# csteinmetz1/dasp-pytorch

Hardware: NVIDIA H100
Metric: audio samples/sec (fwd+bwd) @ batch=1024x2chx48k (higher is better)
Workload: dtype f32

## Files before the change

### dasp_pytorch_b200/csrc/reverb.cu

```cuda
#include <cufft.h>
#include <curand_kernel.h>
#include <math.h>

#include <map>
#include <mutex>
#include <tuple>
#include <vector>

#include "common.cuh"
#include "fft8192.cuh"

namespace dasp {
namespace {

constexpr int kBands = 12;
constexpr int kB = 4096;
constexpr int kNbA = 2 * kB;
constexpr double kPi = 3.14159265358979323846;

#define DASP_CUFFT_OK(expr)                                                        \
  do {                                                                             \
    cufftResult r__ = (expr);                                                      \
    if (r__ != CUFFT_SUCCESS) {                                                    \
      ::dasp::set_error("%s failed: cufft error %d (%s:%d)", #expr, (int)r__, __FILE__, __LINE__); \
// ... 784 lines not shown
  FftSmem s(sm);
  __shared__ float red[kFusedThreads / 32][2 * kBands];
  __shared__ float rk[kBands];
  __shared__ int cls_lo[17], cls_off[17];
  const int t = threadIdx.x;
  s.init(twiddles, t);
  const fft8k::Tables tb = fft8k::carve_tables(s.tabf);
  auto fetch = [&](int it, int m) {
    if (t != 0 || m >= nunits) return;
    uint64_t* bar = &s.full[it & 1];
    float* dst = s.G + (it & 1) * 2 * fft8k::kPlaneG;
    const float* src = Epl + (int64_t)m * 2 * kNbA;
    mbar_arrive_expect_tx(bar, 2u * kNbA * 4u);
#pragma unroll
    for (int q = 0; q < 4; ++q) tma_load_1d(dst + q * 4096, src + q * 4096, 16384u, bar);
  };
  fetch(0, blockIdx.x);
  fetch(1, blockIdx.x + gridDim.x);
  const float step = 1.0f / (float)(L - 1);
  float2* D = reinterpret_cast<float2*>(s.Yr);
  int it = 0;
  for (int m = blockIdx.x; m < nunits; m += gridDim.x, ++it) {
    mbar_wait(&s.full[it & 1], (uint32_t)((it >> 1) & 1));
    float* gr = s.G + (it & 1) * 2 * fft8k::kPlaneG;
    const int64_t il = m / J;
    const int j = m - (int)il * J;
    const int lo = j * kB, hi = (lo + kB < leff) ? lo + kB : leff;
    float xr[16], xi[16];
    fft8192_in_smem<true>(gr, gr + fft8k::kPlaneG, s, tb, t, [&] { fetch(it + 2, m + 2 * gridDim.x); }, [] {}, xr, xi);
    __syncthreads();
    if (t < kBands) rk[t] = -(params[il * 25 + kBands + t] * 10.0f + 1.0f);
    if (t == 0) {
      int off = 0;
      for (int c = 0; c < R; ++c) {
        const int a_lo = (lo - c + R - 1) / R, a_hi = (hi - c + R - 1) / R;
        cls_lo[c] = a_lo;
        cls_off[c] = off;
        off += (a_hi > a_lo) ? a_hi - a_lo : 0;
      }
      cls_off[R] = off;
    }
#pragma unroll
    for (int q = 0; q < 8; ++q) D[t + 512 * q] = make_float2(xr[q], xi[q]);
    __syncthreads();
    float s0[kBands], s1[kBands];
#pragma unroll
    for (int k = 0; k < kBands; ++k) { s0[k] = 0.f; s1[k] = 0.f; }
    const float2* cb = C + (il * kBands) * (int64_t)R * nb;
    const int ntaps = cls_off[R];
    for (int idx = t; idx < ntaps; idx += kFusedThreads) {
      int c = 0;
      while (c + 1 < R && idx >= cls_off[c + 1]) ++c;
      const int a = cls_lo[c] + (idx - cls_off[c]);
      const int tau = R * a + c;
      const float2 gd = D[tau - lo];
      const float tt = time_axis32(tau, L, step);
      const float2* c0 = cb + (int64_t)c * nb + a;
      float2 v[kBands];
#pragma unroll
      for (int k = 0; k < kBands; ++k) v[k] = c0[(int64_t)k * R * nb];
#pragma unroll
      for (int k = 0; k < kBands; ++k) {
        const float w = fmaf(gd.x, v[k].x, gd.y * v[k].y) * __expf(rk[k] * tt);
        s0[k] += w;
        s1[k] = fmaf(w, tt, s1[k]);
      }
    }
    const int lane = t & 31, warp = t >> 5;
#pragma unroll
    for (int k = 0; k < kBands; ++k) {
      const float x0 = warp_sum(s0[k]), x1 = warp_sum(s1[k]);
      if (lane == 0) { red[warp][2 * k] = x0; red[warp][2 * k + 1] = x1; }
    }
    __syncthreads();
    if (t < 2 * kBands) {
      float acc = 0.f;
#pragma unroll
      for (int w = 0; w < kFusedThreads / 32; ++w) acc += red[w][t];
      part[((int64_t)m * kBands) * 2 + t] = acc;
    }
  }
}

constexpr int kMaxFusedR = 8;

__device__ __forceinline__ unsigned cluster_ctarank() {
  unsigned r;
  asm volatile("mov.u32 %0, %%cluster_ctarank;" : "=r"(r));
  return r;
}
__device__ __forceinline__ void cluster_arrive() { asm volatile("barrier.cluster.arrive.release;" ::: "memory"); }
__device__ __forceinline__ void cluster_wait() { asm volatile("barrier.cluster.wait.acquire;" ::: "memory"); }
__device__ __forceinline__ float* map_to_cta(float* smem_ptr, unsigned rank) {
  uint64_t r;
  asm volatile("mapa.u64 %0, %1, %2;" : "=l"(r) : "l"(reinterpret_cast<uint64_t>(smem_ptr)), "r"(rank));
  return reinterpret_cast<float*>(r);
}

template <int R>
__global__ void __launch_bounds__(kFusedThreads, 1)
ir_synth_fused_kernel(const float2* __restrict__ H1, const float* __restrict__ twiddles,
                      const float* __restrict__ params, float2* __restrict__ Hb, float2* __restrict__ Csave, int64_t item0, int64_t L, int64_t leff, int jb,
                      const unsigned long long* seed) {
  constexpr int nb = fft8k::kN, U = nb / 2 + 1, CT = R * kFusedThreads, total = kBands * U;
  static_assert(CT < U, "at most one band may complete per generation round");
  extern __shared__ __align__(16) float sm[];
  float* G = sm;
  float* Yr = sm + 4 * fft8k::kPlaneG;
  float* Yi = Yr + fft8k::kPlaneY;
  float* tabf = Yi + fft8k::kPlaneY;
  float* gk = tabf + fft8k::kTabFloats;
  float* rk = gk + 16;
  const int t = threadIdx.x;
  const unsigned c = cluster_ctarank();
  const int64_t il = blockIdx.y;

  for (int e = t; e < fft8k::kTabFloats; e += kFusedThreads) tabf[e] = twiddles[e];
  if (t < kBands) {
    gk[t] = params[il * 25 + t] * (1.0f / kBands);
    rk[t] = -(params[il * 25 + kBands + t] * 10.0f + 1.0f);
  }
  const fft8k::Tables tb = fft8k::carve_tables(tabf);
  float* remote[R];
#pragma unroll
  for (int b = 0; b < R; ++b) remote[b] = map_to_cta(G, (unsigned)b);
  const PhiloxKeys keys = philox_keys(__ldg(seed));
  const float step = 1.0f / (float)(L - 1);
  float accr[16], acci[16];
#pragma unroll
  for (int q = 0; q < 16; ++q) { accr[q] = 0.f; acci[q] = 0.f; }
  cluster_arrive();
  cluster_wait();

  int processed = 0;
  bool buffer_handed_back = false;
  constexpr int rounds = (total + CT - 1) / CT;
  for (int r = 0; r < rounds; ++r) {
    if (buffer_handed_back) { cluster_wait(); buffer_handed_back = false; }
    const int u = r * CT + (int)c * kFusedThreads + t;
    if (u < total) {
      const int k = u / U, j1 = u - k * U;
      const unsigned long long pair = (unsigned long long)((item0 + il) * kBands + k);
      const bool self_mirror = (j1 == 0) || (2 * j1 == nb);
      const int off = (k & 1) * 2 * fft8k::kPlaneG;
      spectral_unit<R>(j1, nb, H1 + (int64_t)k * (R * nb / 2 + 1), pair, keys, [&](int b, float2 q, float2 qm) {
        float* base = remote[b] + off;
        base[j1] = q.x;
        base[fft8k::kPlaneG + j1] = q.y;
        if (!self_mirror) {
          base[nb - j1] = qm.x;
          base[fft8k::kPlaneG + nb - j1] = qm.y;
        }
      });
    }
    const int done = (r + 1) * CT < total ? (r + 1) * CT : total;
    if (done / U > processed) {
      cluster_arrive();
      cluster_wait();
      const int kk = processed;
      float* gr = G + (kk & 1) * 2 * fft8k::kPlaneG;
      float* gi = gr + fft8k::kPlaneG;
      fft8k::p1<true>(gr, gi, tb, t);
      __syncthreads();
      fft8k::p2<true>(gr, gi, Yr, Yi, tb, t);
      __syncthreads();
      cluster_arrive();
      buffer_handed_back = true;
      fft8k::P3Regs q3;
      fft8k::p3_load<true>(Yr, Yi, t, q3);
      __syncthreads();
      fft8k::p3_store<true>(Yr, Yi, tb, t, q3);
      __syncthreads();
      float xr[16], xi[16];
      fft8k::p4<true>(Yr, Yi, t, xr, xi);
      const float g = gk[kk], rr = rk[kk];
      float2* fout = Csave ? Csave + ((il * kBands + kk) * R + c) * (int64_t)nb : nullptr;
#pragma unroll
      for (int q = 0; q < 16; ++q) {
        const int a = t + 512 * q;
        const float e = g * __expf(rr * time_axis((int64_t)R * a + c, L, step));
        accr[q] = fmaf(e, xr[q], accr[q]);
        acci[q] = fmaf(e, xi[q], acci[q]);
        if (fout) fout[a] = make_float2(xr[q], xi[q]);
      }
      ++processed;
    }
  }
  if (buffer_handed_back) cluster_wait();
  float2* out = Hb + il * (int64_t)jb * kNbA;
#pragma unroll
  for (int q = 0; q < 16; ++q) {
    const int64_t tau = (int64_t)R * (t + 512 * q) + c;
    if (tau < leff) out[(tau / kB) * kNbA + (tau % kB)] = make_float2(accr[q], acci[q]);
  }
}

__global__ void ir_grad_pp_kernel(const float2* __restrict__ Et, const float2* __restrict__ C,
                                  const float* __restrict__ params, float* __restrict__ part, int64_t L, int64_t leff,
                                  int jb, int R, int nb) {
  const int64_t il = blockIdx.y;
  __shared__ float rk[kBands];
  __shared__ float red[8][2 * kBands];
  if (threadIdx.x < kBands) rk[threadIdx.x] = -(params[il * 25 + kBands + threadIdx.x] * 10.0f + 1.0f);
  __syncthreads();
  const float step = 1.0f / (float)(L - 1);
  const float2* de = Et + il * (int64_t)jb * kNbA;
  const float2* cb = C + (il * kBands) * (int64_t)R * nb;
  float s0[kBands], s1[kBands];
#pragma unroll
  for (int k = 0; k < kBands; ++k) { s0[k] = 0.f; s1[k] = 0.f; }
  const int stride = gridDim.x * blockDim.x;
  for (int t = blockIdx.x * blockDim.x + threadIdx.x; t < leff; t += 2 * stride) {
    const int t2 = t + stride;
    const bool has2 = t2 < leff;
    const int a = t / R, ph = t - a * R;
    const int a2 = has2 ? t2 / R : a, ph2 = has2 ? t2 - a2 * R : ph;
    const float2 gd = de[(t / kB) * kNbA + (t % kB)];
    const float2 gd2 = has2 ? de[(t2 / kB) * kNbA + (t2 % kB)] : make_float2(0.f, 0.f);
    const float2* c0 = cb + (int64_t)ph * nb + a;
    const float2* c1 = cb + (int64_t)ph2 * nb + a2;
    float2 v[kBands], v2[kBands];
#pragma unroll
    for (int k = 0; k < kBands; ++k) { v[k] = c0[(int64_t)k * R * nb]; v2[k] = c1[(int64_t)k * R * nb]; }
    const float tt = time_axis(t, L, step), tt2 = time_axis(has2 ? t2 : t, L, step);
#pragma unroll
    for (int k = 0; k < kBands; ++k) {
      const float w = fmaf(gd.x, v[k].x, gd.y * v[k].y) * __expf(rk[k] * tt);
      const float w2 = fmaf(gd2.x, v2[k].x, gd2.y * v2[k].y) * __expf(rk[k] * tt2);
      s0[k] += w + w2;
      s1[k] = fmaf(w, tt, fmaf(w2, tt2, s1[k]));
    }
  }
  const int lane = threadIdx.x & 31, warp = threadIdx.x >> 5;
#pragma unroll
  for (int k = 0; k < kBands; ++k) {
    const float x0 = warp_sum(s0[k]), x1 = warp_sum(s1[k]);
    if (lane == 0) { red[warp][2 * k] = x0; red[warp][2 * k + 1] = x1; }
  }
  __syncthreads();
  if (threadIdx.x < 2 * kBands) {
    float acc = 0.f;
    for (int w = 0; w < (int)(blockDim.x >> 5); ++w) acc += red[w][threadIdx.x];
    part[((il * gridDim.x + blockIdx.x) * kBands) * 2 + threadIdx.x] = acc;
  }
}


__global__ void x_blocks_kernel(const float* __restrict__ x, float2* __restrict__ Xb, int64_t item0, int I, int64_t n,
                                int in_chs) {
  const int i = blockIdx.x;
  const int64_t il = blockIdx.y;
  const float* xl = x + ((item0 + il) * in_chs) * n;
  const float* xr = in_chs == 1 ? xl : xl + n;
  float2* out = Xb + (il * I + i) * (int64_t)kNbA;
  for (int m = threadIdx.x; m < kNbA; m += blockDim.x) {
    const int64_t idx = (int64_t)(i - 1) * kB + m;
    float2 v = make_float2(0.f, 0.f);
    if (idx >= 0 && idx < n) v = make_float2(xl[idx], xr[idx]);
    out[m] = v;
  }
}

__device__ __forceinline__ void untangle(float2 z, float2 zm, float2& a, float2& b) {
  a = make_float2(0.5f * (z.x + zm.x), 0.5f * (z.y - zm.y));
  b = make_float2(0.5f * (z.y + zm.y), -0.5f * (z.x - zm.x));
}
__device__ __forceinline__ void cfma(float2& acc, float2 p, float2 q) {
  acc.x = fmaf(p.x, q.x, fmaf(-p.y, q.y, acc.x));
  acc.y = fmaf(p.x, q.y, fmaf(p.y, q.x, acc.y));
}
__device__ __forceinline__ void cfma_conj(float2& acc, float2 p, float2 q) {
  acc.x = fmaf(p.x, q.x, fmaf(p.y, q.y, acc.x));
  acc.y = fmaf(p.y, q.x, fmaf(-p.x, q.y, acc.y));
}

template <int MAXB, bool CORR, bool PLANAR = false>
__global__ void __launch_bounds__(128) partition_mac_kernel(const float2* __restrict__ A, const float2* __restrict__ Bm,
// ... 372 lines not shown
  for (int k = 0; k < kBands; ++k)
    for (int64_t i = 0; i < g.taps; ++i) padded[(size_t)k * n1 + i] = taps[(size_t)k * g.taps + i] * inv;
  float* d_in = nullptr;
  cufftComplex* d_out = nullptr;
  void* d_work = nullptr;
  DASP_CUDA_OK(cudaMalloc(&d_in, sizeof(float) * padded.size()));
  DASP_CUDA_OK(cudaMalloc(&d_out, sizeof(cufftComplex) * kBands * n1c));
  DASP_CUDA_OK(cudaMemcpyAsync(d_in, padded.data(), sizeof(float) * padded.size(), cudaMemcpyHostToDevice, st));
  PlanVal pv;
  int rc = get_plan(0, n1, kBands, n1, n1c, pv);
  if (rc != DASP_OK) return rc;
  DASP_CUDA_OK(cudaMalloc(&d_work, pv.work > 0 ? pv.work : 16));
  DASP_CUFFT_OK(cufftSetStream(pv.h, st));
  DASP_CUFFT_OK(cufftSetWorkArea(pv.h, d_work));
  DASP_CUFFT_OK(cufftExecR2C(pv.h, d_in, d_out));
  DASP_CUDA_OK(cudaStreamSynchronize(st));
  cudaFree(d_in);
  cudaFree(d_work);
  g_fb[key] = d_out;
  *out = reinterpret_cast<const float2*>(d_out);
  return DASP_OK;
}

template <int R>
void launch_spectral(float2* C, const float2* H1, int64_t item0, int64_t items, int nb, const unsigned long long* seed,
                     bool planar, cudaStream_t st) {
  const int threads = 128;
  dim3 grid((unsigned)((nb / 2 + 1 + threads - 1) / threads), kBands, (unsigned)items);
  if (planar) spectral_gen_kernel<R, true><<<grid, threads, 0, st>>>(C, H1, item0, nb, seed);
  else        spectral_gen_kernel<R, false><<<grid, threads, 0, st>>>(C, H1, item0, nb, seed);
}
bool dispatch_spectral(int R, float2* C, const float2* H1, int64_t item0, int64_t items, int nb,
                       const unsigned long long* seed, bool planar, cudaStream_t st) {
  switch (R) {
#define DASP_R(r) case r: launch_spectral<r>(C, H1, item0, items, nb, seed, planar, st); return true;
    DASP_R(1) DASP_R(2) DASP_R(3) DASP_R(4) DASP_R(5) DASP_R(6) DASP_R(7) DASP_R(8) DASP_R(9) DASP_R(10)
    DASP_R(11) DASP_R(12) DASP_R(13) DASP_R(14) DASP_R(15) DASP_R(16)
#undef DASP_R
    default: return false;
  }
}
constexpr int kMaxSpectralR = 16;

std::map<int, float*> g_fft_tab;
int get_fft_tables(cudaStream_t st, const float** out) {
  int dev = 0;
  DASP_CUDA_OK(cudaGetDevice(&dev));
  auto it = g_fft_tab.find(dev);
  if (it == g_fft_tab.end()) {
    std::vector<float> h(fft8k::kTabFloats, 0.f);
    for (int e = 0; e < fft8k::kTabEntries; ++e) {
      int co, so, dup;
      double turns;
      fft8k::table_entry(e, co, so, dup, turns);
      const float c = (float)cos(2.0 * kPi * turns), sn = (float)sin(2.0 * kPi * turns);
      h[co] = c; h[so] = sn;
      if (dup) { h[co + 1] = c; h[so + 1] = sn; }
    }
    float* d = nullptr;
    DASP_CUDA_OK(cudaMalloc(&d, sizeof(float) * h.size()));
    DASP_CUDA_OK(cudaMemcpyAsync(d, h.data(), sizeof(float) * h.size(), cudaMemcpyHostToDevice, st));
    DASP_CUDA_OK(cudaStreamSynchronize(st));
    it = g_fft_tab.emplace(dev, d).first;
  }
  *out = it->second;
  return DASP_OK;
}
int configure_fft_kernels();
int launch_ifft_shape(float2* C, const float* tw, const float* params, float2* hs, bool save_f, int64_t items,
                      const Geom& g, int jb, cudaStream_t st) {
  int rc = configure_fft_kernels();
  if (rc != DASP_OK) return rc;
  const size_t smem = kFftSmemBytes;
  ifft_shape_kernel<<<dim3((unsigned)g.rpp, (unsigned)items), kFusedThreads, smem, st>>>(
      reinterpret_cast<float*>(C), tw, params, hs, save_f ? 1 : 0, (int)g.L, (int)g.leff, jb, (int)g.rpp);
  DASP_LAUNCH_OK("ifft_shape_kernel");
  return DASP_OK;
}
int g_last_fused = 0;
std::map<std::pair<int, int>, int> g_fused_ok;
template <int R>
bool launch_fused(const float2* H1, const float* tw, const float* params, float2* hs, float2* Csave, int64_t item0, int64_t items,
                  int64_t L, int64_t leff, int jb, const unsigned long long* seed, cudaStream_t st) {
  auto kern = ir_synth_fused_kernel<R>;
  const size_t smem = sizeof(float) * kFusedSmemFloats;
  cudaLaunchConfig_t cfg = {};
  cfg.gridDim = dim3(R, (unsigned)items, 1);
  cfg.blockDim = dim3(kFusedThreads, 1, 1);
  cfg.dynamicSmemBytes = smem;
  cfg.stream = st;
  cudaLaunchAttribute at[1];
  at[0].id = cudaLaunchAttributeClusterDimension;
  at[0].val.clusterDim.x = R; at[0].val.clusterDim.y = 1; at[0].val.clusterDim.z = 1;
  cfg.attrs = at;
  cfg.numAttrs = 1;
  int dev = 0;
  cudaGetDevice(&dev);
  auto it = g_fused_ok.find({dev, R});
  if (it == g_fused_ok.end()) {
    int n = 0;
    if (cudaFuncSetAttribute(kern, cudaFuncAttributeMaxDynamicSharedMemorySize, (int)smem) != cudaSuccess ||
        cudaOccupancyMaxActiveClusters(&n, kern, &cfg) != cudaSuccess) {
      n = 0;
      cudaGetLastError();
    }
    it = g_fused_ok.emplace(std::make_pair(dev, R), n).first;
  }
  if (it->second < 1) return false;
  cudaLaunchKernelEx(&cfg, kern, H1, tw, params, hs, Csave, item0, L, leff, jb, seed);
  return true;
}
bool dispatch_fused(int R, const float2* H1, const float* tw, const float* params, float2* hs, float2* Csave, int64_t item0,
                    int64_t items, int64_t L, int64_t leff, int jb, const unsigned long long* seed, cudaStream_t st) {
  switch (R) {
#define DASP_R(r) case r: return launch_fused<r>(H1, tw, params, hs, Csave, item0, items, L, leff, jb, seed, st);
    DASP_R(1) DASP_R(2) DASP_R(3) DASP_R(4) DASP_R(5) DASP_R(6) DASP_R(7) DASP_R(8)
#undef DASP_R
    default: return false;
  }
}

inline size_t align256(size_t v) { return (v + 255) & ~(size_t)255; }

struct FwdWs { size_t ys, xsp, hsp, extra, cufft, total; };
struct BwdWs { size_t gs, ds, es, extra, mixpart, cufft, total; };

void fwd_layout(const ConvGeom& g, size_t extra_bytes, size_t cufft_work, FwdWs& w) {
  size_t o = 0;
  w.ys = o;  o += align256(sizeof(float2) * (size_t)(g.chunk * g.ib * kNbA));
  w.xsp = o; o += align256(sizeof(float2) * (size_t)(g.chunk * g.ib * kNbA));
  w.hsp = o; o += align256(sizeof(float2) * (size_t)(g.chunk * g.jb * kNbA));
  w.extra = o; o += align256(extra_bytes);
  w.cufft = o; o += align256(cufft_work);
  w.total = o;
}
void bwd_layout(const ConvGeom& g, size_t extra_bytes, size_t cufft_work, BwdWs& w) {
  size_t o = 0;
  w.gs = o; o += align256(sizeof(float2) * (size_t)(g.chunk * g.ib * kNbA));
  w.ds = o; o += align256(sizeof(float2) * (size_t)(g.chunk * g.ib * kNbA));
  w.es = o; o += align256(sizeof(float2) * (size_t)(g.chunk * g.jb * kNbA));
  w.extra = o; o += align256(extra_bytes);
  w.mixpart = o; o += align256(sizeof(float) * (size_t)(g.chunk * g.ib));
  w.cufft = o; o += align256(cufft_work);
  w.total = o;
}

struct Plans { PlanVal xi, hj, blk, pp; };
struct Setup { Plans full, rem; FwdWs fwd; BwdWs bwd; };
int conv_setup(const ConvGeom& g, const Geom* synth, Setup& s) {
  int rc;
  size_t work = 0;
  for (int64_t items : {g.bs > 0 ? g.chunk : 0, g.bs % g.chunk}) {
    if (items == 0) continue;
    Plans& p = items == g.chunk ? s.full : s.rem;
    if ((rc = get_plan(2, kNbA, items * g.ib, kNbA, kNbA, p.xi)) != DASP_OK) return rc;
    if ((rc = get_plan(2, kNbA, items * g.jb, kNbA, kNbA, p.hj)) != DASP_OK) return rc;
    if (p.xi.work > work) work = p.xi.work;
    if (p.hj.work > work) work = p.hj.work;
    if (synth) {
      if ((rc = get_plan(2, synth->nb, items * kBands * synth->nbk, synth->nb, synth->nb, p.blk)) != DASP_OK) return rc;
      if ((rc = get_plan(2, synth->nb, items * kBands * synth->rpp, synth->nb, synth->nb, p.pp)) != DASP_OK) return rc;
      if (p.blk.work > work) work = p.blk.work;
      if (p.pp.work > work) work = p.pp.work;
    }
  }
  size_t fwd_extra = 0, bwd_extra = 0;
  if (synth) {
    fwd_extra = sizeof(float2) * (size_t)(g.chunk * kBands * synth->pair_c64());
    int64_t nparts = synth->nbk > synth->nparts_pp() ? synth->nbk : synth->nparts_pp();
    if (g.jb > nparts) nparts = g.jb;
    bwd_extra = sizeof(float) * (size_t)(g.chunk * nparts * kBands * 2);
  }
  fwd_layout(g, fwd_extra, work, s.fwd);
  bwd_layout(g, bwd_extra, work, s.bwd);
  return DASP_OK;
}
int check_workspace(const char* what, size_t need, int64_t have) {
  if ((int64_t)need > have) {
    set_error("%s: workspace needs %lld bytes, got %lld", what, (long long)need, (long long)have);
    return DASP_ERR_WORKSPACE;
  }
  return DASP_OK;
}

template <class Out>
int put_conv_geometry(const ConvGeom& g, const Geom* synth, Out* out) {
  std::lock_guard<std::mutex> lk(g_mu);
  Setup s{};
  int rc = conv_setup(g, synth, s);
  if (rc != DASP_OK) return rc;
  out->leff = g.leff; out->conv_block = kB; out->x_blocks = g.ib; out->ir_partitions = g.jb; out->chunk_items = g.chunk;
  out->xspec_c64 = g.bs * g.ib * kNbA;
  out->irspec_c64 = g.bs * g.jb * kNbA;
  out->fwd_workspace_bytes = (int64_t)s.fwd.total;
  out->bwd_workspace_bytes = (int64_t)s.bwd.total;
  return DASP_OK;
}

template <bool CORR, bool PLANAR = false>
// ... 132 lines not shown
}

}

void reverb_shutdown() {
  std::lock_guard<std::mutex> lk(g_mu);
  for (auto& kv : g_plans) cufftDestroy(kv.second.h);
  g_plans.clear();
  for (auto& kv : g_fb) cudaFree(kv.second);
  g_fb.clear();
  for (auto& kv : g_fft_tab) cudaFree(kv.second);
  g_fft_tab.clear();
}

}

using namespace dasp;

extern "C" {

int dasp_debug_reverb_last_path(void) { return g_last_fused; }

int dasp_reverb_filterbank(int64_t taps, double sample_rate, float* out) {
  DASP_REQUIRE(out != nullptr && taps >= 1 && (taps % 2) == 1, "filterbank: taps must be odd and out non-null");
  DASP_REQUIRE(sample_rate / 2.0 > 18000.0, "filterbank: needs 18 kHz < sample_rate/2");
  std::vector<float> v;
  octave_filterbank((int)taps, sample_rate, v);
  for (size_t i = 0; i < v.size(); ++i) out[i] = v[i];
  return DASP_OK;
}

int dasp_reverb_geometry(int64_t bs, int64_t n, int64_t num_samples, int64_t taps, int64_t chunk_items,
                         dasp_reverb_geom* out) {
  DASP_REQUIRE(out != nullptr, "reverb geometry: null out");
  Geom g;
  int rc = make_geom(bs, n, num_samples, taps, chunk_items, g);
  if (rc != DASP_OK) return rc;
  if ((rc = put_conv_geometry(g, &g, out)) != DASP_OK) return rc;
  out->nb = g.nb; out->hop = g.hop; out->nbk = g.nbk; out->rpp = g.rpp;
  out->f_floats = bs * kBands * g.pair_c64() * 2;
  return DASP_OK;
}

int dasp_reverb_fwd(const float* x, int64_t in_chs, const float* params, const float* noise, const uint64_t* seed_dev, float* y,
                    float* f_save, void* xspec_save, void* irspec_save, void* workspace,
                    int64_t workspace_bytes, int64_t bs, int64_t n, int64_t num_samples, int64_t taps,
                    int64_t chunk_items, float sample_rate, void* stream) {
  Geom g;
  int rc = make_geom(bs, n, num_samples, taps, chunk_items, g);
  if (rc != DASP_OK) return rc;
  DASP_REQUIRE(in_chs == 1 || in_chs == 2, "only mono/stereo signals are supported");
  if (bs == 0) return DASP_OK;
  DASP_REQUIRE(x && params && y && workspace, "reverb fwd: null pointer");
  DASP_REQUIRE(noise != nullptr || seed_dev != nullptr, "reverb fwd: device-noise mode needs seed_dev (a device pointer)");
  const unsigned long long* seed = reinterpret_cast<const unsigned long long*>(seed_dev);
  cudaStream_t st = (cudaStream_t)stream;
  std::lock_guard<std::mutex> lk(g_mu);
  const float2 *H = nullptr, *H1 = nullptr;
  const bool spectral = (noise == nullptr) && g.rpp <= kMaxSpectralR;
  if (spectral) { if ((rc = get_filterbank_n1(g, (double)sample_rate, st, &H1)) != DASP_OK) return rc; }
  else          { if ((rc = get_filterbank(g, (double)sample_rate, st, &H)) != DASP_OK) return rc; }
  Setup s{};
  if ((rc = conv_setup(g, &g, s)) != DASP_OK) return rc;
  if ((rc = check_workspace("reverb fwd", s.fwd.total, workspace_bytes)) != DASP_OK) return rc;
  const FwdWs& w = s.fwd;
  unsigned char* base = (unsigned char*)workspace;
  void* ws_cufft = base + w.cufft;
  const int64_t lp = g.L + g.P;
  const int nbk = (int)g.nbk, nb = (int)g.nb, hop = (int)g.hop, P = (int)g.P, I = (int)g.ib, J = (int)g.jb;

  for (int64_t item0 = 0; item0 < bs; item0 += g.chunk) {
    const int64_t items = (bs - item0 < g.chunk) ? bs - item0 : g.chunk;
    const Plans& pl = (items == g.chunk) ? s.full : s.rem;
    float2* C = f_save ? reinterpret_cast<float2*>(f_save) + item0 * kBands * g.pair_c64()
                       : reinterpret_cast<float2*>(base + w.extra);
    float2* xs = xspec_save ? (float2*)xspec_save + item0 * I * (int64_t)kNbA : (float2*)(base + w.xsp);
    float2* hs = irspec_save ? (float2*)irspec_save + item0 * J * (int64_t)kNbA : (float2*)(base + w.hsp);
    const dim3 gblk((unsigned)nbk, kBands, (unsigned)items);
    const bool own_conv = own_fft_rows(n, x, hs);

    if (!own_conv) DASP_CUDA_OK(cudaMemsetAsync(hs, 0, sizeof(float2) * items * J * kNbA, st));
    int synth = 0;
    const bool own_fft = spectral && nb == fft8k::kN && g.L < (int64_t)1 << 31;
    if (own_fft && debug_reverb_path() == 2 && g.rpp <= kMaxFusedR) synth = 1;
    else if (own_fft && debug_reverb_path() != 1) synth = 2;
    const float* tw = nullptr;
    if ((synth != 0 || own_conv) && (rc = get_fft_tables(st, &tw)) != DASP_OK) return rc;
    if (synth == 1) {
      if (dispatch_fused((int)g.rpp, H1, tw, params + item0 * 25, hs, f_save ? C : nullptr, item0, items, g.L, g.leff, J,
                         seed, st)) {
        DASP_LAUNCH_OK("ir_synth_fused_kernel");
      } else {
        synth = 2;
      }
    }
    g_last_fused = synth;
    if (synth == 1) {
    } else if (synth == 2) {
      dispatch_spectral((int)g.rpp, C, H1, item0, items, nb, seed, true, st);
      DASP_LAUNCH_OK("spectral_gen_kernel");
      if ((rc = launch_ifft_shape(C, tw, params + item0 * 25, hs, f_save != nullptr, items, g, J, st)) != DASP_OK) return rc;
    } else if (spectral) {
      dispatch_spectral((int)g.rpp, C, H1, item0, items, nb, seed, false, st);
      DASP_LAUNCH_OK("spectral_gen_kernel");
      DASP_CUFFT_OK(cufftSetStream(pl.pp.h, st));
      DASP_CUFFT_OK(cufftSetWorkArea(pl.pp.h, ws_cufft));
      DASP_CUFFT_OK(cufftExecC2C(pl.pp.h, (cufftComplex*)C, (cufftComplex*)C, CUFFT_INVERSE));
      shape_ir_pp_kernel<<<dim3((unsigned)((g.leff + 255) / 256), (unsigned)items), 256, 0, st>>>(
          C, params + item0 * 25, hs, g.L, g.leff, J, (int)g.rpp, nb);
      DASP_LAUNCH_OK("shape_ir_pp_kernel");
    } else {
      if (noise) noise_pairs_layout_kernel<<<gblk, 256, 0, st>>>(noise, C, item0, nbk, nb, hop, lp);
      else       noise_pairs_philox_kernel<<<gblk, 256, 0, st>>>(C, item0, nbk, nb, hop, seed);
      DASP_LAUNCH_OK("reverb noise kernel");
      DASP_CUFFT_OK(cufftSetStream(pl.blk.h, st));
      DASP_CUFFT_OK(cufftSetWorkArea(pl.blk.h, ws_cufft));
      DASP_CUFFT_OK(cufftExecC2C(pl.blk.h, (cufftComplex*)C, (cufftComplex*)C, CUFFT_FORWARD));
      cmul_filter_pairs_kernel<<<gblk, 256, 0, st>>>(C, H, nbk, nb);
      DASP_LAUNCH_OK("cmul_filter_pairs_kernel");
      DASP_CUFFT_OK(cufftExecC2C(pl.blk.h, (cufftComplex*)C, (cufftComplex*)C, CUFFT_INVERSE));
      shape_ir_pairs_kernel<<<dim3((unsigned)nbk, (unsigned)items), 256, 0, st>>>(C, params + item0 * 25, hs, g.L, g.leff,
                                                                               J, nbk, nb, hop, P);
      DASP_LAUNCH_OK("shape_ir_pairs_kernel");
    }
    if ((rc = conv_fwd_chunk(g, pl, own_conv, tw, x, (int)in_chs, xs, hs, params + 24, 25, y, base, w, item0, items,
                             st)) != DASP_OK)
      return rc;
  }
  return DASP_OK;
}

int dasp_reverb_bwd(const float* gy, const float* x, int64_t in_chs, const float* params,
                    const float* f_save, const void* xspec_save, const void* irspec_save, float* gx, float* gparams,
                    void* workspace, int64_t workspace_bytes, int64_t bs, int64_t n, int64_t num_samples, int64_t taps,
                    int64_t chunk_items, int64_t device_noise, void* stream) {
  Geom g;
  int rc = make_geom(bs, n, num_samples, taps, chunk_items, g);
  if (rc != DASP_OK) return rc;
  DASP_REQUIRE(in_chs == 1 || in_chs == 2, "only mono/stereo signals are supported");
  if (bs == 0) return DASP_OK;
  const bool polyphase = device_noise != 0 && g.rpp <= kMaxSpectralR;
  DASP_REQUIRE(gy && x && params && f_save && xspec_save && irspec_save && gx && gparams && workspace,
               "reverb bwd: null pointer");
  cudaStream_t st = (cudaStream_t)stream;
  std::lock_guard<std::mutex> lk(g_mu);
  Setup s{};
  if ((rc = conv_setup(g, &g, s)) != DASP_OK) return rc;
  if ((rc = check_workspace("reverb bwd", s.bwd.total, workspace_bytes)) != DASP_OK) return rc;
  const BwdWs& w = s.bwd;
  unsigned char* base = (unsigned char*)workspace;
  const float2* ws_es = (const float2*)(base + w.es);
  float* ws_irpart = (float*)(base + w.extra);
  const float* ws_mixpart = (const float*)(base + w.mixpart);
  const int nbk = (int)g.nbk, nb = (int)g.nb, hop = (int)g.hop, P = (int)g.P, I = (int)g.ib, J = (int)g.jb;

  for (int64_t item0 = 0; item0 < bs; item0 += g.chunk) {
    const int64_t items = (bs - item0 < g.chunk) ? bs - item0 : g.chunk;
    const Plans& pl = (items == g.chunk) ? s.full : s.rem;
    const float2* C = reinterpret_cast<const float2*>(f_save) + item0 * kBands * g.pair_c64();
    const float2* xs = (const float2*)xspec_save + item0 * I * (int64_t)kNbA;
    const float2* hs = (const float2*)irspec_save + item0 * J * (int64_t)kNbA;

    const bool own_conv = own_fft_rows(n, gy, nullptr);
    const bool own_irgrad = own_conv && polyphase && nb == fft8k::kN && g.L < (int64_t)1 << 31;
    const float* tw = nullptr;
    if (own_conv && (rc = get_fft_tables(st, &tw)) != DASP_OK) return rc;
    if ((rc = conv_bwd_chunk(g, pl, own_conv, own_irgrad ? IrGrad::kPlanar : IrGrad::kTime, tw, gy, x, (int)in_chs, xs,
                             hs, params + 24, 25, gx, base, w, item0, items, st)) != DASP_OK)
      return rc;
    int nparts;
    if (own_irgrad) {
      nparts = J;
      const int nunits = (int)(items * J);
      const unsigned ig_grid = (unsigned)(nunits < sm_count() ? nunits : sm_count());
      ifft_irgrad_kernel<<<ig_grid, kFusedThreads, kFftSmemBytes, st>>>(reinterpret_cast<const float*>(ws_es), tw, C,
                                                                        params + item0 * 25, ws_irpart, (int)g.L,
                                                                        (int)g.leff, J, (int)g.rpp, nunits);
      DASP_LAUNCH_OK("ifft_irgrad_kernel");
    } else {
      if (polyphase) {
        nparts = (int)g.nparts_pp();
// ... 123 lines not shown
```

Measured before the change: 4.560 billion.

## Warp-specialize cluster IR synthesis with async remote stores and mbarrier double-buffering

Replaces the fused IR synthesis kernel with a warp-specialized cluster kernel. Dedicated generator warps, with reduced registers via setmaxnreg, write spectral bins into peer CTAs' shared memory using st.async with mbarrier transaction counts. FFT warps consume double-buffered bands signalled by full/empty mbarriers instead of cluster-wide barriers, and the kernel is persistent across items with the grid capped by max active clusters. It also replaces per-element expf with a recurrence for the decay envelope. It becomes the default path for rpp<=6 instead of the two-kernel spectral+iFFT path, which adds complexity and occupancy risk.

```diff
diff --git a/dasp_pytorch_b200/csrc/reverb.cu b/dasp_pytorch_b200/csrc/reverb.cu
--- a/dasp_pytorch_b200/csrc/reverb.cu
+++ b/dasp_pytorch_b200/csrc/reverb.cu
@@ -890,117 +890,173 @@
   }
 }
 
-constexpr int kMaxFusedR = 8;
-
+constexpr int kMaxClusterR = 6;
+constexpr int kSynthGen = 384, kSynthThreads = kFusedThreads + kSynthGen;
+constexpr int kSynthFftRegs = 80, kSynthGenRegs = 56;
+constexpr int kMaxHookR = 8;
+constexpr size_t kSynthSmemBytes =
+    sizeof(float) * (2 * 2 * fft8k::kPlaneG + 2 * fft8k::kPlaneY + fft8k::kTabFloats) + 4 * sizeof(uint64_t);
+
+__device__ __forceinline__ void cluster_arrive() { asm volatile("barrier.cluster.arrive.release;" ::: "memory"); }
+__device__ __forceinline__ void cluster_wait() { asm volatile("barrier.cluster.wait.acquire;" ::: "memory"); }
 __device__ __forceinline__ unsigned cluster_ctarank() {
   unsigned r;
   asm volatile("mov.u32 %0, %%cluster_ctarank;" : "=r"(r));
   return r;
 }
-__device__ __forceinline__ void cluster_arrive() { asm volatile("barrier.cluster.arrive.release;" ::: "memory"); }
-__device__ __forceinline__ void cluster_wait() { asm volatile("barrier.cluster.wait.acquire;" ::: "memory"); }
-__device__ __forceinline__ float* map_to_cta(float* smem_ptr, unsigned rank) {
-  uint64_t r;
-  asm volatile("mapa.u64 %0, %1, %2;" : "=l"(r) : "l"(reinterpret_cast<uint64_t>(smem_ptr)), "r"(rank));
-  return reinterpret_cast<float*>(r);
-}
+__device__ __forceinline__ uint32_t mapa_u32(uint32_t smem_addr, uint32_t rank) {
+  uint32_t r;
+  asm("mapa.shared::cluster.u32 %0, %1, %2;" : "=r"(r) : "r"(smem_addr), "r"(rank));
+  return r;
+}
+__device__ __forceinline__ void st_async(uint32_t addr, float v, uint32_t bar) {
+  asm volatile("st.async.shared::cluster.mbarrier::complete_tx::bytes.b32 [%0], %1, [%2];" ::"r"(addr),
+               "r"(__float_as_uint(v)), "r"(bar)
+               : "memory");
+}
+__device__ __forceinline__ void mbar_arrive_remote(uint32_t cluster_bar) {
+  asm volatile("mbarrier.arrive.relaxed.cluster.shared::cluster.b64 _, [%0];" ::"r"(cluster_bar) : "memory");
+}
+__device__ __forceinline__ void fence_cluster() { asm volatile("fence.acq_rel.cluster;" ::: "memory"); }
+__device__ __forceinline__ void mbar_wait_cluster(uint64_t* bar, uint32_t parity) {
+  uint32_t done;
+  do {
+    asm volatile(
+        "{\n.reg .pred p;\n"
+        "mbarrier.try_wait.parity.acquire.cluster.shared::cta.b64 p, [%1], %2;\n"
+        "selp.u32 %0, 1, 0, p;\n}\n"
+        : "=r"(done)
+        : "r"(smem_u32(bar)), "r"(parity)
+        : "memory");
+  } while (!done);
+}
+__device__ __forceinline__ void fft_sync() { asm volatile("bar.sync 1, %0;" ::"n"(kFusedThreads) : "memory"); }
 
 template <int R>
-__global__ void __launch_bounds__(kFusedThreads, 1)
-ir_synth_fused_kernel(const float2* __restrict__ H1, const float* __restrict__ twiddles,
-                      const float* __restrict__ params, float2* __restrict__ Hb, float2* __restrict__ Csave, int64_t item0, int64_t L, int64_t leff, int jb,
-                      const unsigned long long* seed) {
-  constexpr int nb = fft8k::kN, U = nb / 2 + 1, CT = R * kFusedThreads, total = kBands * U;
-  static_assert(CT < U, "at most one band may complete per generation round");
-  extern __shared__ __align__(16) float sm[];
+__global__ void __launch_bounds__(kSynthThreads, 1)
+ir_synth_cluster_kernel(const float2* __restrict__ H1, const float* __restrict__ twiddles, const float* __restrict__ params,
+                        float2* __restrict__ Hb, float2* __restrict__ Csave, int64_t item0, int items, int L, int leff,
+                        int jb, const unsigned long long* seed) {
+  constexpr int nb = fft8k::kN, U = nb / 2 + 1, NG = kSynthGen, NT = kSynthThreads;
+  constexpr int CT = R * NG, total = kBands * U;
+  constexpr uint32_t kBandBytes = 2u * nb * 4u;
+  extern __shared__ __align__(128) float sm[];
   float* G = sm;
   float* Yr = sm + 4 * fft8k::kPlaneG;
   float* Yi = Yr + fft8k::kPlaneY;
   float* tabf = Yi + fft8k::kPlaneY;
-  float* gk = tabf + fft8k::kTabFloats;
-  float* rk = gk + 16;
+  uint64_t* full = reinterpret_cast<uint64_t*>(tabf + fft8k::kTabFloats);
+  uint64_t* empty = full + 2;
   const int t = threadIdx.x;
   const unsigned c = cluster_ctarank();
-  const int64_t il = blockIdx.y;
-
-  for (int e = t; e < fft8k::kTabFloats; e += kFusedThreads) tabf[e] = twiddles[e];
-  if (t < kBands) {
-    gk[t] = params[il * 25 + t] * (1.0f / kBands);
-    rk[t] = -(params[il * 25 + kBands + t] * 10.0f + 1.0f);
-  }
-  const fft8k::Tables tb = fft8k::carve_tables(tabf);
-  float* remote[R];
-#pragma unroll
-  for (int b = 0; b < R; ++b) remote[b] = map_to_cta(G, (unsigned)b);
-  const PhiloxKeys keys = philox_keys(__ldg(seed));
-  const float step = 1.0f / (float)(L - 1);
-  float accr[16], acci[16];
-#pragma unroll
-  for (int q = 0; q < 16; ++q) { accr[q] = 0.f; acci[q] = 0.f; }
+  const int my_items = items > (int)blockIdx.y ? (items - 1 - (int)blockIdx.y) / (int)gridDim.y + 1 : 0;
+  const int nbands = my_items * kBands;
+
+  for (int e = t; e < fft8k::kTabFloats; e += NT) tabf[e] = twiddles[e];
+  if (t == 0) {
+    mbar_init(&full[0], 1);
+    mbar_init(&full[1], 1);
+    mbar_init(&empty[0], R);
+    mbar_init(&empty[1], R);
+    fence_barrier_init();
+    if (nbands > 0) mbar_arrive_expect_tx(&full[0], kBandBytes);
+    if (nbands > 1) mbar_arrive_expect_tx(&full[1], kBandBytes);
+  }
+  __syncthreads();
   cluster_arrive();
   cluster_wait();
 
-  int processed = 0;
-  bool buffer_handed_back = false;
-  constexpr int rounds = (total + CT - 1) / CT;
-  for (int r = 0; r < rounds; ++r) {
-    if (buffer_handed_back) { cluster_wait(); buffer_handed_back = false; }
-    const int u = r * CT + (int)c * kFusedThreads + t;
-    if (u < total) {
-      const int k = u / U, j1 = u - k * U;
-      const unsigned long long pair = (unsigned long long)((item0 + il) * kBands + k);
-      const bool self_mirror = (j1 == 0) || (2 * j1 == nb);
-      const int off = (k & 1) * 2 * fft8k::kPlaneG;
-      spectral_unit<R>(j1, nb, H1 + (int64_t)k * (R * nb / 2 + 1), pair, keys, [&](int b, float2 q, float2 qm) {
-        float* base = remote[b] + off;
-        base[j1] = q.x;
-        base[fft8k::kPlaneG + j1] = q.y;
-        if (!self_mirror) {
-          base[nb - j1] = qm.x;
-          base[fft8k::kPlaneG + nb - j1] = qm.y;
+  if (t >= kFusedThreads) {
+    asm volatile("setmaxnreg.dec.sync.aligned.u32 %0;" ::"n"(kSynthGenRegs));
+    const int gt = t - kFusedThreads;
+    const PhiloxKeys keys = philox_keys(__ldg(seed));
+    const uint32_t g_local = smem_u32(G), full_local = smem_u32(full);
+    int waited = 1;
+    for (int i = 0; i < my_items; ++i) {
+      const int64_t il = blockIdx.y + (int64_t)i * gridDim.y;
+      for (int u = (int)c * NG + gt; u < total; u += CT) {
+        const int k = u / U, j1 = u - k * U;
+        const int g = i * kBands + k;
+        if (g > waited) {
+          mbar_wait_cluster(&empty[k & 1], (uint32_t)(((g - 2) >> 1) & 1));
+          waited = g;
         }
-      });
-    }
-    const int done = (r + 1) * CT < total ? (r + 1) * CT : total;
-    if (done / U > processed) {
-      cluster_arrive();
-      cluster_wait();
-      const int kk = processed;
-      float* gr = G + (kk & 1) * 2 * fft8k::kPlaneG;
-      float* gi = gr + fft8k::kPlaneG;
-      fft8k::p1<true>(gr, gi, tb, t);
-      __syncthreads();
-      fft8k::p2<true>(gr, gi, Yr, Yi, tb, t);
-      __syncthreads();
-      cluster_arrive();
-      buffer_handed_back = true;
-      fft8k::P3Regs q3;
-      fft8k::p3_load<true>(Yr, Yi, t, q3);
-      __syncthreads();
-      fft8k::p3_store<true>(Yr, Yi, tb, t, q3);
-      __syncthreads();
-      float xr[16], xi[16];
-      fft8k::p4<true>(Yr, Yi, t, xr, xi);
-      const float g = gk[kk], rr = rk[kk];
-      float2* fout = Csave ? Csave + ((il * kBands + kk) * R + c) * (int64_t)nb : nullptr;
+        const unsigned long long pair = (unsigned long long)((item0 + il) * kBands + k);
+        const bool self_mirror = (j1 == 0) || (2 * j1 == nb);
+        const uint32_t off = (uint32_t)(k & 1) * kBandBytes;
+        spectral_unit<R>(j1, nb, H1 + (int64_t)k * (R * nb / 2 + 1), pair, keys, [&](int b, float2 q, float2 qm) {
+          const uint32_t base = mapa_u32(g_local + off, (uint32_t)b);
+          const uint32_t bar = mapa_u32(full_local + 8u * (uint32_t)(k & 1), (uint32_t)b);
+          st_async(base + 4u * j1, q.x, bar);
+          st_async(base + 4u * (fft8k::kPlaneG + j1), q.y, bar);
+          if (!self_mirror) {
+            st_async(base + 4u * (nb - j1), qm.x, bar);
+            st_async(base + 4u * (fft8k::kPlaneG + nb - j1), qm.y, bar);
+          }
+        });
+      }
+    }
+  } else {
+    asm volatile("setmaxnreg.inc.sync.aligned.u32 %0;" ::"n"(kSynthFftRegs));
+    const fft8k::Tables tb = fft8k::carve_tables(tabf);
+    const float step = 1.0f / (float)(L - 1);
+    for (int i = 0; i < my_items; ++i) {
+      const int64_t il = blockIdx.y + (int64_t)i * gridDim.y;
+      float accr[16], acci[16];
+#pragma unroll
+      for (int q = 0; q < 16; ++q) { accr[q] = 0.f; acci[q] = 0.f; }
+      for (int k = 0; k < kBands; ++k) {
+        const int g = i * kBands + k;
+        if (t < 32) mbar_wait_cluster(&full[k & 1], (uint32_t)((g >> 1) & 1));
+        fft_sync();
+        float* gr = G + (k & 1) * 2 * fft8k::kPlaneG;
+        float* gi = gr + fft8k::kPlaneG;
+        fft8k::p1<true>(gr, gi, tb, t);
+        fft_sync();
+        fft8k::p2<true>(gr, gi, Yr, Yi, tb, t);
+        fence_proxy_async_smem();
+        fft_sync();
+        if (t == 0 && g + 2 < nbands) {
+          mbar_arrive_expect_tx(&full[k & 1], kBandBytes);
+          fence_cluster();
+#pragma unroll
+          for (int b = 0; b < R; ++b) {
+            mbar_arrive_remote(mapa_u32(smem_u32(&empty[k & 1]), (uint32_t)b));
+          }
+        }
+        fft8k::P3Regs q3;
+        fft8k::p3_load<true>(Yr, Yi, t, q3);
+        fft_sync();
+        fft8k::p3_store<true>(Yr, Yi, tb, t, q3);
+        fft_sync();
+        float xr[16], xi[16];
+        fft8k::p4<true>(Yr, Yi, t, xr, xi);
+        float e_prev = 0.f;
+        const float g_k = params[il * 25 + k] * (1.0f / kBands), rr = -(params[il * 25 + kBands + k] * 10.0f + 1.0f);
+        float2* fout = Csave ? Csave + ((il * kBands + k) * R + c) * (int64_t)nb : nullptr;
+        const float rho = __expf(rr * step * (float)(512 * R));
+#pragma unroll
+        for (int q = 0; q < 16; ++q) {
+          const int a = t + 512 * q;
+          float e;
+          if ((q & 3) == 0) e = g_k * __expf(rr * time_axis32(R * a + (int)c, L, step));
+          else e = e_prev * rho;
+          e_prev = e;
+          accr[q] = fmaf(e, xr[q], accr[q]);
+          acci[q] = fmaf(e, xi[q], acci[q]);
+          if (fout) fout[a] = make_float2(xr[q], xi[q]);
+        }
+      }
+      float2* out = Hb + il * (int64_t)jb * kNbA;
 #pragma unroll
       for (int q = 0; q < 16; ++q) {
-        const int a = t + 512 * q;
-        const float e = g * __expf(rr * time_axis((int64_t)R * a + c, L, step));
-        accr[q] = fmaf(e, xr[q], accr[q]);
-        acci[q] = fmaf(e, xi[q], acci[q]);
-        if (fout) fout[a] = make_float2(xr[q], xi[q]);
+        const int tau = R * (t + 512 * q) + (int)c;
+        if (tau < leff) out[(tau / kB) * kNbA + (tau % kB)] = make_float2(accr[q], acci[q]);
       }
-      ++processed;
-    }
-  }
-  if (buffer_handed_back) cluster_wait();
-  float2* out = Hb + il * (int64_t)jb * kNbA;
-#pragma unroll
-  for (int q = 0; q < 16; ++q) {
-    const int64_t tau = (int64_t)R * (t + 512 * q) + c;
-    if (tau < leff) out[(tau / kB) * kNbA + (tau % kB)] = make_float2(accr[q], acci[q]);
-  }
+    }
+  }
+  cluster_arrive();
+  cluster_wait();
 }
 
 __global__ void ir_grad_pp_kernel(const float2* __restrict__ Et, const float2* __restrict__ C,
@@ -1539,12 +1595,10 @@
 template <int R>
 bool launch_fused(const float2* H1, const float* tw, const float* params, float2* hs, float2* Csave, int64_t item0, int64_t items,
                   int64_t L, int64_t leff, int jb, const unsigned long long* seed, cudaStream_t st) {
-  auto kern = ir_synth_fused_kernel<R>;
-  const size_t smem = sizeof(float) * kFusedSmemFloats;
+  auto kern = ir_synth_cluster_kernel<R>;
   cudaLaunchConfig_t cfg = {};
-  cfg.gridDim = dim3(R, (unsigned)items, 1);
-  cfg.blockDim = dim3(kFusedThreads, 1, 1);
-  cfg.dynamicSmemBytes = smem;
+  cfg.blockDim = dim3(kSynthThreads, 1, 1);
+  cfg.dynamicSmemBytes = kSynthSmemBytes;
   cfg.stream = st;
   cudaLaunchAttribute at[1];
   at[0].id = cudaLaunchAttributeClusterDimension;
@@ -1556,7 +1610,8 @@
   auto it = g_fused_ok.find({dev, R});
   if (it == g_fused_ok.end()) {
     int n = 0;
-    if (cudaFuncSetAttribute(kern, cudaFuncAttributeMaxDynamicSharedMemorySize, (int)smem) != cudaSuccess ||
+    cfg.gridDim = dim3(R, 1, 1);
+    if (cudaFuncSetAttribute(kern, cudaFuncAttributeMaxDynamicSharedMemorySize, (int)kSynthSmemBytes) != cudaSuccess ||
         cudaOccupancyMaxActiveClusters(&n, kern, &cfg) != cudaSuccess) {
       n = 0;
       cudaGetLastError();
@@ -1564,14 +1619,16 @@
     it = g_fused_ok.emplace(std::make_pair(dev, R), n).first;
   }
   if (it->second < 1) return false;
-  cudaLaunchKernelEx(&cfg, kern, H1, tw, params, hs, Csave, item0, L, leff, jb, seed);
+  const int64_t clusters = items < it->second ? items : it->second;
+  cfg.gridDim = dim3(R, (unsigned)clusters, 1);
+  cudaLaunchKernelEx(&cfg, kern, H1, tw, params, hs, Csave, item0, (int)items, (int)L, (int)leff, jb, seed);
   return true;
 }
 bool dispatch_fused(int R, const float2* H1, const float* tw, const float* params, float2* hs, float2* Csave, int64_t item0,
                     int64_t items, int64_t L, int64_t leff, int jb, const unsigned long long* seed, cudaStream_t st) {
   switch (R) {
 #define DASP_R(r) case r: return launch_fused<r>(H1, tw, params, hs, Csave, item0, items, L, leff, jb, seed, st);
-    DASP_R(1) DASP_R(2) DASP_R(3) DASP_R(4) DASP_R(5) DASP_R(6) DASP_R(7) DASP_R(8)
+    DASP_R(1) DASP_R(2) DASP_R(3) DASP_R(4) DASP_R(5) DASP_R(6)
 #undef DASP_R
     default: return false;
   }
@@ -1870,21 +1927,19 @@
     if (!own_conv) DASP_CUDA_OK(cudaMemsetAsync(hs, 0, sizeof(float2) * items * J * kNbA, st));
     int synth = 0;
     const bool own_fft = spectral && nb == fft8k::kN && g.L < (int64_t)1 << 31;
-    if (own_fft && debug_reverb_path() == 2 && g.rpp <= kMaxFusedR) synth = 1;
-    else if (own_fft && debug_reverb_path() != 1) synth = 2;
+    const bool two_kernel_hook = debug_reverb_path() == 2 && g.rpp <= kMaxHookR;
+    if (own_fft && debug_reverb_path() != 1) synth = two_kernel_hook ? 1 : 2;
     const float* tw = nullptr;
     if ((synth != 0 || own_conv) && (rc = get_fft_tables(st, &tw)) != DASP_OK) return rc;
-    if (synth == 1) {
-      if (dispatch_fused((int)g.rpp, H1, tw, params + item0 * 25, hs, f_save ? C : nullptr, item0, items, g.L, g.leff, J,
-                         seed, st)) {
-        DASP_LAUNCH_OK("ir_synth_fused_kernel");
-      } else {
-        synth = 2;
-      }
-    }
     g_last_fused = synth;
-    if (synth == 1) {
-    } else if (synth == 2) {
+    bool clustered = false;
+    if (synth == 2 && g.rpp <= kMaxClusterR) {
+      clustered = dispatch_fused((int)g.rpp, H1, tw, params + item0 * 25, hs, f_save ? C : nullptr, item0, items, g.L,
+                                 g.leff, J, seed, st);
+      if (clustered) DASP_LAUNCH_OK("ir_synth_cluster_kernel");
+    }
+    if (clustered) {
+    } else if (synth != 0) {
       dispatch_spectral((int)g.rpp, C, H1, item0, items, nb, seed, true, st);
       DASP_LAUNCH_OK("spectral_gen_kernel");
       if ((rc = launch_ifft_shape(C, tw, params + item0 * 25, hs, f_save != nullptr, items, g, J, st)) != DASP_OK) return rc;
```

After: 4.839 billion, median of 6. 1.06x the previous value.
